# OPPO-Mente-Lab/X2I

Measured on AMD Instinct MI355X. Metric: images/sec, FLUX-schnell 1024x1024 4-step (projector + denoise loop), whole job, higher is better.
Workload: dtype bf16; 1 GPU; BASELINE configs[1]: qwen3b conditioning (C=37,H=2048,S_txt=512) -> projector -> shuttle-3/FLUX-schnell DiT 1024x1024, 4 steps; batch_per_gpu=4, global_batch=4, parallelism=batch-sharded x1, graph=True

## Files before the change

### x2i_amd/csrc/c_api.hip

```cpp
#include <stdarg.h>
#include <stdio.h>

#include "x2i_common.h"
#include "x2i_kernels.h"

static thread_local char g_err[512] = "";

int x2i_set_error(int code, const char* fmt, ...) {
  va_list ap;
  va_start(ap, fmt);
  vsnprintf(g_err, sizeof(g_err), fmt, ap);
  va_end(ap);
  return code;
}

int x2i_check_launch(const char* what) {
  hipError_t e = hipGetLastError();
  if (e != hipSuccess) return x2i_set_error(X2I_ERR_HIP, "%s: launch failed: %s", what, hipGetErrorString(e));
  return X2I_OK;
}

#include <stdlib.h>
#include <string.h>

#include <mutex>
#include <set>
#include <utility>

namespace {
int env_int(const char* name, int dflt) {
  const char* v = getenv(name);
  return v && *v ? atoi(v) : dflt;
}
X2IOptions make_options() {
  X2IOptions o;
  o.gemm_tile = env_int("X2I_GEMM_TILE", 0);
  o.gemm_min256 = env_int("X2I_GEMM_MIN256", 128);
  o.gemm_gm = env_int("X2I_GEMM_GM", 0);
  o.gemm_split_tail = env_int("X2I_GEMM_NOSPLIT", 0) ? 0 : 1;
  o.gemm_w4 = env_int("X2I_GEMM_W4", 1);
  o.gemm_persist = env_int("X2I_GEMM_PERSIST", 1);
  o.gemm_fp8_persist = env_int("X2I_GEMM_FP8_PERSIST", 1);
  o.gemm_fx = env_int("X2I_GEMM_FX", 2);
  o.gemm_fx_nk = env_int("X2I_GEMM_FX_NK", 96);
  o.gemm_streamk = env_int("X2I_GEMM_STREAMK", 1);
  o.gemm_pair = env_int("X2I_GEMM_PAIR", 1);
  o.train_rows_wg = env_int("X2I_TRAIN_ROWS_WG", 1);
  o.attn_bwd_overlap = env_int("X2I_ATTN_BWD_OVERLAP", 1);
  o.conv256 = env_int("X2I_CONV256", 1);
  o.conv_w4 = env_int("X2I_CONV_W4", 1);
  o.conv_korder = env_int("X2I_CONV_KORDER", 1);
  o.attn_variant = env_int("X2I_ATTN_VARIANT", 0);
  o.attn_w16 = env_int("X2I_ATTN_W16", 1);
  o.attn_streamk = env_int("X2I_ATTN_STREAMK", 1);
  o.conv5_variant = env_int("X2I_CONV5_VARIANT", 0);
  o.fp8 = env_int("X2I_FP8", 0);
  o.last_gemm_tile = X2I_FORM_NONE;
  o.attn_ablate = env_int("X2I_ATTN_ABLATE", 0);
  return o;
}
std::mutex g_smem_mu;
std::set<std::pair<const void*, int>> g_smem_done;
}

X2IOptions& x2i_options() {
  static X2IOptions o = make_options();
  return o;
}

int x2i_ensure_dynamic_smem(const void* kernel, int bytes) {
  int dev = 0;
  hipGetDevice(&dev);
  const std::pair<const void*, int> key(kernel, dev);
  std::lock_guard<std::mutex> lk(g_smem_mu);
  if (g_smem_done.count(key)) return X2I_OK;
  const hipError_t e = hipFuncSetAttribute(kernel, hipFuncAttributeMaxDynamicSharedMemorySize, bytes);
  if (e != hipSuccess) return x2i_set_error(X2I_ERR_HIP, "hipFuncSetAttribute(MaxDynamicSharedMemorySize=%d): %s", bytes, hipGetErrorString(e));
  g_smem_done.insert(key);
  return X2I_OK;
}

int x2i_num_cus() {
  static int cus[64] = {0};
  int dev = 0;
  hipGetDevice(&dev);
  if (dev < 0 || dev >= 64) dev = 0;
  if (!cus[dev]) {
    int n = 0;
    if (hipDeviceGetAttribute(&n, hipDeviceAttributeMultiprocessorCount, dev) != hipSuccess || n <= 0) n = 256;
    cus[dev] = n;
  }
  return cus[dev];
}

bool x2i_streamk_workspace(const x2i_gemm_args* a, float** slabs, unsigned** flags, int* rc) {
  *rc = X2I_OK;
  if (!a->workspace) return false;
  const long long need = 4096 + (long long)x2i_gemm_sk_slabs() * x2i_gemm_sk_slab_bytes();
  if (a->workspace_bytes < need || (((uintptr_t)a->workspace) & 255)) {
    *rc = x2i_set_error(X2I_ERR_ARG, "gemm: stream-K workspace must be 256-byte aligned and >= x2i_streamk_workspace_bytes() = %lld bytes (got %lld)",
                        need, (long long)a->workspace_bytes);
    return false;
  }
  *flags = (unsigned*)a->workspace;
  *slabs = (float*)((char*)a->workspace + 4096);
  return true;
}

extern "C" {

int x2i_abi_version(void) { return X2I_ABI_VERSION; }

static long long* opt_slot(X2IOptions& o, const char* name, int** as_int) {
  *as_int = nullptr;
#define X2I_OPT_INT(N_) if (!strcmp(name, #N_)) { *as_int = &o.N_; return nullptr; }
  X2I_OPT_INT(gemm_tile) X2I_OPT_INT(gemm_gm) X2I_OPT_INT(gemm_split_tail) X2I_OPT_INT(gemm_w4) X2I_OPT_INT(gemm_persist) X2I_OPT_INT(gemm_fp8_persist) X2I_OPT_INT(gemm_fx) X2I_OPT_INT(gemm_fx_nk) X2I_OPT_INT(gemm_streamk) X2I_OPT_INT(gemm_pair) X2I_OPT_INT(train_rows_wg) X2I_OPT_INT(attn_bwd_overlap) X2I_OPT_INT(attn_streamk) X2I_OPT_INT(conv256) X2I_OPT_INT(conv_w4) X2I_OPT_INT(conv_korder) X2I_OPT_INT(attn_variant) X2I_OPT_INT(attn_w16) X2I_OPT_INT(conv5_variant) X2I_OPT_INT(fp8) X2I_OPT_INT(last_gemm_tile)
#ifdef X2I_ABLATION
  X2I_OPT_INT(attn_ablate)
#endif
#undef X2I_OPT_INT
  if (!strcmp(name, "gemm_min256")) return &o.gemm_min256;
  return nullptr;
}

int x2i_set_option(const char* name, int64_t value) {
  if (!name) return x2i_set_error(X2I_ERR_ARG, "set_option: null name");
  int* ip;
  long long* lp = opt_slot(x2i_options(), name, &ip);
  if (ip) *ip = (int)value;
  else if (lp) *lp = (long long)value;
  else return x2i_set_error(X2I_ERR_ARG, "set_option: unknown option '%s'", name);
  return X2I_OK;
}

int x2i_get_option(const char* name, int64_t* value) {
  if (!name || !value) return x2i_set_error(X2I_ERR_ARG, "get_option: null pointer");
  int* ip;
  long long* lp = opt_slot(x2i_options(), name, &ip);
  if (ip) *value = *ip;
  else if (lp) *value = *lp;
  else return x2i_set_error(X2I_ERR_ARG, "get_option: unknown option '%s'", name);
  return X2I_OK;
}

int64_t x2i_streamk_workspace_bytes(void) { return 4096 + (int64_t)x2i_gemm_sk_slabs() * x2i_gemm_sk_slab_bytes(); }

int x2i_streamk_workspace_status(const void* workspace, int64_t workspace_bytes) {
  if (!workspace || workspace_bytes < x2i_streamk_workspace_bytes()) return x2i_set_error(X2I_ERR_ARG, "streamk_workspace_status: no / too small workspace");
  unsigned v = 0;
  const hipError_t e = hipMemcpy(&v, (const unsigned*)workspace + x2i_gemm_sk_max_tiles(), 4, hipMemcpyDeviceToHost);
  if (e != hipSuccess) return x2i_set_error(X2I_ERR_HIP, "streamk_workspace_status: %s", hipGetErrorString(e));
  return v ? 1 : 0;
}

int x2i_is_ablation_build(void) {
#ifdef X2I_ABLATION
  return 1;
#else
  return 0;
#endif
}
const char* x2i_last_error(void) { return g_err; }

int x2i_gemm_bf16(const x2i_gemm_args* args, x2i_stream_t stream) { return x2i_launch_gemm(args, (hipStream_t)stream); }

int x2i_gemm_fp8(const x2i_gemm_args* args, const x2i_fp8_desc* fp8, x2i_stream_t stream) {
  return x2i_launch_gemm_fp8(args, fp8, (hipStream_t)stream);
}

// ... 340 lines not shown
```

### x2i_amd/csrc/elementwise.hip

```cpp
#include "x2i_common.h"
#include "x2i_kernels.h"

namespace {

__device__ __forceinline__ void unpack8(const bf16x8_t& v, float (&f)[8]) {
#pragma unroll
  for (int i = 0; i < 8; ++i) f[i] = bf16_to_f32((bf16_t)v[i]);
}
__device__ __forceinline__ bf16x8_t pack8(const float (&f)[8]) {
  union { bf16x8_t v; uint32_t u[4]; } r;
#pragma unroll
  for (int i = 0; i < 4; ++i) r.u[i] = pack_bf16x2(f[2 * i], f[2 * i + 1]);
  return r.v;
}

constexpr int LN_MAXV = 8;

template <bool AFFINE>
__global__ __launch_bounds__(256) void ln_kernel(const bf16_t* __restrict__ X, long long x_bs, int ldx, bf16_t* __restrict__ Y,
                                                 long long y_bs, int ldy, int S, int D, int S0, const float* shift0,
                                                 const float* scale0, const float* shift1, const float* scale1,
                                                 long long mod_bs, const bf16_t* aw, const bf16_t* ab, float eps,
                                                 long long total_rows) {
  const int lane = threadIdx.x & 63;
// ... 223 lines not shown
#pragma unroll
      for (int b = 0; b < NB; ++b) acc[r][b] = 0.f;
#pragma unroll
      for (int q = 0; q < NP; ++q) acc2[r][q] = f32x2{0.f, 0.f};
    }
    for (int k = lane * 8; k < K; k += 512) {
      bf16x8_t wv[R];
#pragma unroll
      for (int r = 0; r < R; ++r) {
        const int n = min(n0 + r, N - 1);
        wv[r] = __builtin_nontemporal_load((const bf16x8_t*)(W + (long long)n * K + k));
      }
      float wf[R][8];
#pragma unroll
      for (int r = 0; r < R; ++r) unpack8(wv[r], wf[r]);
#pragma unroll
      for (int j = 0; j < 8; ++j) {
        const float* xk = xs + (k + j) * NBP;
#pragma unroll
        for (int q = 0; q < NP; ++q) {
          const f32x2 x2 = *(const f32x2*)(xk + 2 * q);
#pragma unroll
          for (int r = 0; r < R; ++r) acc2[r][q] = __builtin_elementwise_fma(f32x2{wf[r][j], wf[r][j]}, x2, acc2[r][q]);
        }
        if constexpr (NB & 1) {
          const float x1 = xk[NB - 1];
#pragma unroll
          for (int r = 0; r < R; ++r) acc[r][NB - 1] = fmaf(wf[r][j], x1, acc[r][NB - 1]);
        }
      }
    }
#pragma unroll
    for (int r = 0; r < R; ++r)
#pragma unroll
      for (int q = 0; q < NP; ++q) { acc[r][2 * q] = acc2[r][q][0]; acc[r][2 * q + 1] = acc2[r][q][1]; }
#pragma unroll
    for (int r = 0; r < R; ++r) {
#pragma unroll
      for (int b = 0; b < NB; ++b) acc[r][b] = wave_sum(acc[r][b]);
      const int n = n0 + r;
      if (lane == 0 && n < N && rr + r < rpw) {
        const float bv = bias ? bf16_to_f32(bias[n]) : 0.f;
#pragma unroll
        for (int b = 0; b < NB; ++b) {
          float v = apply_act(acc[r][b] + bv, act_out);
          float* yp = Y + (long long)b * ldy + n;
          *yp = accumulate ? (*yp + v) : v;
        }
      }
    }
  }
}

__global__ void sinusoid_kernel(const float* __restrict__ t, float* __restrict__ out, int B, int dim, int round_bf16) {
  const int i = blockIdx.x * blockDim.x + threadIdx.x;
  const int half = dim / 2;
  if (i >= B * dim) return;
  const int b = i / dim, j = i - b * dim;
  const int k = j < half ? j : j - half;
  const float f = expf(-logf(10000.f) * (float)k / (float)half);
  const float a = t[b] * f;
  float v = j < half ? cosf(a) : sinf(a);
  if (round_bf16) v = bf16_to_f32(f32_to_bf16(v));
  out[i] = v;
}

__global__ void rope_table_kernel(const float* __restrict__ ids, int S, int d0, int d1, int d2, double theta, float* __restrict__ cosp,
                                  float* __restrict__ sinp) {
  const int D = d0 + d1 + d2;
  const long long i = (long long)blockIdx.x * blockDim.x + threadIdx.x;
  if (i >= (long long)S * D) return;
  const int s = (int)(i / D), c = (int)(i - (long long)s * D);
  int a = 0, start = 0, d = d0;
  if (c >= d0 + d1) a = 2, start = d0 + d1, d = d2;
  else if (c >= d0) a = 1, start = d0, d = d1;
  const int k = (c - start) >> 1;
  const double freq = 1.0 / pow(theta, (double)(2 * k) / (double)d);
  const double ang = (double)ids[(long long)s * 3 + a] * freq;
  cosp[i] = (float)cos(ang);
  sinp[i] = (float)sin(ang);
}

__global__ void euler_kernel(bf16_t* __restrict__ x, const bf16_t* __restrict__ eps, long long n8, const float* __restrict__ dt) {
  const float d = dt[0];
  for (long long i = (long long)blockIdx.x * blockDim.x + threadIdx.x; i < n8; i += (long long)gridDim.x * blockDim.x) {
    float a[8], e[8];
    unpack8(*(const bf16x8_t*)(x + i * 8), a);
    unpack8(*(const bf16x8_t*)(eps + i * 8), e);
#pragma unroll
    for (int j = 0; j < 8; ++j) a[j] = a[j] + d * e[j];
    *(bf16x8_t*)(x + i * 8) = pack8(a);
  }
}

__global__ __launch_bounds__(256) void gated_residual_kernel(bf16_t* __restrict__ X, long long x_bs, int ldx, const bf16_t* __restrict__ T,
                                                             long long t_bs, int ldt, const float* __restrict__ gate, long long g_bs, int S,
                                                             int D8, long long total) {
  for (long long i = (long long)blockIdx.x * blockDim.x + threadIdx.x; i < total; i += (long long)gridDim.x * blockDim.x) {
    const int c = (int)(i % D8);
    const long long row = i / D8;
    const int b = (int)(row / S), s = (int)(row - (long long)b * S);
    bf16_t* x = X + (long long)b * x_bs + (long long)s * ldx + c * 8;
    float a[8], t[8];
    unpack8(*(const bf16x8_t*)x, a);
    unpack8(*(const bf16x8_t*)(T + (long long)b * t_bs + (long long)s * ldt + c * 8), t);
    const float* g = gate + (long long)b * g_bs + c * 8;
// ... 38 lines not shown
  if (ldx % 8 || ldy % 8 || x_bs % 8 || y_bs % 8 || mod_bs % 4 || !al16(X) || !al16(Y)) return x2i_set_error(X2I_ERR_ALIGN, "ln_modulate: rows must be 16-byte aligned");
  const long long rows = (long long)B * S;
  if (D == 3072 && rows >= 4096) {
    hipLaunchKernelGGL((ln_rows_kernel<6, 4>), dim3((unsigned)((rows + 15) / 16)), dim3(256), 0, stream, (const bf16_t*)X, x_bs, ldx, (bf16_t*)Y, y_bs,
                       ldy, S, S0, shift0 ? shift0 : shift1, scale0 ? scale0 : scale1, shift1, scale1, mod_bs, eps, rows);
    return x2i_check_launch("ln_modulate");
  }
  hipLaunchKernelGGL(ln_kernel<false>, dim3((unsigned)((rows + 3) / 4)), dim3(256), 0, stream, (const bf16_t*)X, x_bs, ldx,
                     (bf16_t*)Y, y_bs, ldy, S, D, S0, shift0 ? shift0 : shift1, scale0 ? scale0 : scale1, shift1, scale1, mod_bs,
                     (const bf16_t*)nullptr, (const bf16_t*)nullptr, eps, rows);
  return x2i_check_launch("ln_modulate");
}

int x2i_launch_ln_affine(const void* X, void* Y, long long rows, int D, const void* w, const void* b, float eps, hipStream_t stream) {
  if (!X || !Y || !w || !b) return x2i_set_error(X2I_ERR_ARG, "ln_affine: null pointer");
  if (D % 8 || D > 64 * 8 * LN_MAXV || rows <= 0) return x2i_set_error(X2I_ERR_SHAPE, "ln_affine: D=%d unsupported", D);
  if (!al16(X) || !al16(Y) || !al16(w) || !al16(b)) return x2i_set_error(X2I_ERR_ALIGN, "ln_affine: 16-byte alignment required");
  hipLaunchKernelGGL(ln_kernel<true>, dim3((unsigned)((rows + 3) / 4)), dim3(256), 0, stream, (const bf16_t*)X, (long long)0, D,
                     (bf16_t*)Y, (long long)0, D, (int)1 << 30, D, 0, (const float*)nullptr, (const float*)nullptr,
                     (const float*)nullptr, (const float*)nullptr, (long long)0, (const bf16_t*)w, (const bf16_t*)b, eps, rows);
  return x2i_check_launch("ln_affine");
}

int x2i_launch_qkv_split(const void* qkv0, const void* qkv1, int ld0, int ld1, int B, int S, int S0, int H, const void* nq0,
                         const void* nk0, const void* nq1, const void* nk1, const float* cosp, const float* sinp, void* Q,
                         void* K, void* VT, int Spad, float eps, hipStream_t stream) {
  if (S0 < 0 || S0 > S || B <= 0 || S <= 0 || H <= 0) return x2i_set_error(X2I_ERR_SHAPE, "qkv_split: bad shape");
  if ((S0 > 0 && (!qkv0 || !nq0 || !nk0)) || (S0 < S && (!qkv1 || !nq1 || !nk1)) || !cosp || !sinp || !Q || !K || !VT)
    return x2i_set_error(X2I_ERR_ARG, "qkv_split: null pointer");
  if (Spad % 128 || Spad < S) return x2i_set_error(X2I_ERR_SHAPE, "qkv_split: Spad=%d must be a multiple of 128 and >= S=%d", Spad, S);
  if ((S0 > 0 && ld0 % 8) || (S0 < S && ld1 % 8)) return x2i_set_error(X2I_ERR_ALIGN, "qkv_split: ld must be a multiple of 8");
  hipLaunchKernelGGL(qk_norm_rope_kernel, dim3(S, B), dim3(256), 0, stream, (const bf16_t*)qkv0, (const bf16_t*)qkv1, ld0, ld1, S,
                     S0, H, (const bf16_t*)nq0, (const bf16_t*)nk0, (const bf16_t*)nq1, (const bf16_t*)nk1, cosp, sinp, (bf16_t*)Q,
                     (bf16_t*)K, Spad, eps);
  int rc = x2i_check_launch("qk_norm_rope");
  if (rc) return rc;
  hipLaunchKernelGGL(v_transpose_kernel, dim3((S + 63) / 64, H, B), dim3(256), 0, stream, (const bf16_t*)qkv0, (const bf16_t*)qkv1,
                     ld0, ld1, S, S0, H, (bf16_t*)VT, Spad);
  return x2i_check_launch("v_transpose");
}

int x2i_launch_skinny_linear(const void* X, int x_is_bf16, const void* W, const void* bias, float* Y, int ldy, int B, int N, int K,
                             int act_in, int act_out, int accumulate, hipStream_t stream) {
  return x2i_launch_skinny_linear_grouped(X, x_is_bf16, 0, W, bias, Y, ldy, 1, B, N, K, act_in, act_out, accumulate, stream);
}

int x2i_launch_skinny_linear_grouped(const void* X, int x_is_bf16, long long x_gs, const void* W, const void* bias, float* Y, int ldy, int G, int B,
                                     int N, int K, int act_in, int act_out, int accumulate, hipStream_t stream) {
  if (!X || !W || !Y) return x2i_set_error(X2I_ERR_ARG, "skinny_linear: null pointer");
  if (G <= 0 || G > 65535 || x_gs < 0) return x2i_set_error(X2I_ERR_SHAPE, "skinny_linear: bad group count / stride (G=%d)", G);
  if (G > 1 && B > SK_MAXB) return x2i_set_error(X2I_ERR_SHAPE, "skinny_linear_grouped: at most %d rows per group (B=%d)", SK_MAXB, B);
  if (B <= 0 || N <= 0 || K <= 0 || K % 8) return x2i_set_error(X2I_ERR_SHAPE, "skinny_linear: K=%d must be a multiple of 8", K);
  if (!al16(W)) return x2i_set_error(X2I_ERR_ALIGN, "skinny_linear: W must be 16-byte aligned");
  const int esz = x_is_bf16 ? 2 : 4;
  for (int b0 = 0; b0 < B; b0 += SK_MAXB) {
    const int nb = (B - b0) < SK_MAXB ? (B - b0) : SK_MAXB;
    const void* xp = (const char*)X + (long long)b0 * K * esz;
    float* yp = Y + (long long)b0 * ldy;
    const int rpw = N >= 65536 ? 16 : 4;
    const dim3 grid((N + 4 * rpw - 1) / (4 * rpw), G), block(256);
    const size_t shm = (size_t)(nb == 1 ? 1 : (nb + 1) & ~1) * K * 4;
    if (shm > 160 * 1024) return x2i_set_error(X2I_ERR_SHAPE, "skinny_linear: B*K too large for LDS");
#define SK_CASE(NB)                                                                                                   \
  case NB: {                                                                                                          \
    hipError_t e = hipFuncSetAttribute((const void*)skinny_linear_kernel<NB>, hipFuncAttributeMaxDynamicSharedMemorySize, \
                                       (int)shm);                                                                     \
    if (e != hipSuccess) return x2i_set_error(X2I_ERR_HIP, "skinny_linear: %s", hipGetErrorString(e));                \
    hipLaunchKernelGGL(skinny_linear_kernel<NB>, grid, block, shm, stream, xp, x_is_bf16, (const bf16_t*)W,           \
                       (const bf16_t*)bias, yp, ldy, N, K, act_in, act_out, accumulate, rpw, x_gs, B);               \
  } break;
    switch (nb) {
      SK_CASE(1) SK_CASE(2) SK_CASE(3) SK_CASE(4) SK_CASE(5) SK_CASE(6) SK_CASE(7) SK_CASE(8)
    }
#undef SK_CASE
    int rc = x2i_check_launch("skinny_linear");
    if (rc) return rc;
  }
  return X2I_OK;
}

int x2i_launch_timestep_sinusoid(const float* t, float* out, int B, int dim, int round_bf16, hipStream_t stream) {
  if (!t || !out || B <= 0 || dim <= 0 || dim % 2) return x2i_set_error(X2I_ERR_ARG, "timestep_sinusoid: bad argument");
  hipLaunchKernelGGL(sinusoid_kernel, dim3((B * dim + 255) / 256), dim3(256), 0, stream, t, out, B, dim, round_bf16);
  return x2i_check_launch("timestep_sinusoid");
}

int x2i_launch_rope_table(const float* ids, int S, int d0, int d1, int d2, float theta, float* cosp, float* sinp, hipStream_t stream) {
  if (!ids || !cosp || !sinp || S <= 0) return x2i_set_error(X2I_ERR_ARG, "rope_table: bad argument");
  if (d0 < 0 || d1 < 0 || d2 < 0 || (d0 | d1 | d2) & 1 || d0 + d1 + d2 <= 0 || theta <= 0.f)
    return x2i_set_error(X2I_ERR_SHAPE, "rope_table: axis dims must be even and non-negative (%d,%d,%d)", d0, d1, d2);
  const long long n = (long long)S * (d0 + d1 + d2);
  hipLaunchKernelGGL(rope_table_kernel, dim3((unsigned)((n + 255) / 256)), dim3(256), 0, stream, ids, S, d0, d1, d2, (double)theta, cosp, sinp);
  return x2i_check_launch("rope_table");
}

int x2i_launch_gated_residual(void* X, long long x_bs, int ldx, const void* T, long long t_bs, int ldt, const float* gate, long long g_bs,
                              int B, int S, int D, hipStream_t stream) {
  if (!X || !T || !gate || B <= 0 || S <= 0 || D <= 0) return x2i_set_error(X2I_ERR_ARG, "gated_residual: bad argument");
  if (D % 8 || ldx % 8 || ldt % 8 || x_bs % 8 || t_bs % 8 || g_bs % 4 || !al16(X) || !al16(T) || !al16(gate))
    return x2i_set_error(X2I_ERR_ALIGN, "gated_residual: rows must be 16-byte aligned, D %% 8 == 0");
  const long long total = (long long)B * S * (D / 8);
  const long long blocks = (total + 255) / 256;
  hipLaunchKernelGGL(gated_residual_kernel, dim3((unsigned)(blocks < 8192 ? blocks : 8192)), dim3(256), 0, stream, (bf16_t*)X, x_bs, ldx,
                     (const bf16_t*)T, t_bs, ldt, gate, g_bs, S, D / 8, total);
  return x2i_check_launch("gated_residual");
}
// ... 36 lines not shown
```

### x2i_amd/csrc/x2i_common.h

```cpp
#pragma once
#include <hip/hip_runtime.h>
#include <stdint.h>

typedef uint16_t bf16_t;
typedef __attribute__((ext_vector_type(8))) short bf16x8_t;
typedef __attribute__((ext_vector_type(4))) short bf16x4_t;
typedef __attribute__((ext_vector_type(4))) float f32x4_t;
typedef __attribute__((ext_vector_type(16))) float f32x16_t;

#define X2I_OK 0
#define X2I_ERR_ARG (-1)
#define X2I_ERR_SHAPE (-2)
#define X2I_ERR_ALIGN (-3)
#define X2I_ERR_HIP (-4)
#define X2I_ERR_STATE (-5)

int x2i_set_error(int code, const char* fmt, ...);
int x2i_check_launch(const char* what);

struct X2IOptions {
  int gemm_tile;
  long long gemm_min256;
  int gemm_gm;
  int gemm_split_tail;
  int gemm_w4;
  int attn_bwd_overlap;
  int train_rows_wg;
  int gemm_pair;
  int gemm_streamk;
  int gemm_fx_nk;
  int gemm_fx;
  int gemm_fp8_persist;
  int gemm_persist;
  int conv256;
  int conv_w4;
  int conv_korder;
  int attn_variant;
  int attn_w16;
  int attn_streamk;
  int conv5_variant;
  int fp8;
  int last_gemm_tile;
  int attn_ablate;
};
X2IOptions& x2i_options();
enum X2IGemmForm {
  X2I_FORM_NONE = -1,
  X2I_FORM_GENERIC = 0,
  X2I_FORM_128 = 128,
  X2I_FORM_256 = 256,
  X2I_FORM_256_TAIL = 1256,
  X2I_FORM_PAIR = 2256,
  X2I_FORM_FX = 3256,
  X2I_FORM_CONV256C = 5256,
  X2I_FORM_CONV512C = 5512,
  X2I_FORM_FP8 = 7256,
  X2I_FORM_FP8_PERSIST = 8256,
  X2I_FORM_FP8_STREAMK = 9256,
};
int x2i_ensure_dynamic_smem(const void* kernel, int bytes);
int x2i_num_cus();
struct x2i_gemm_args;
bool x2i_streamk_workspace(const x2i_gemm_args* a, float** slabs, unsigned** flags, int* rc);
long long x2i_conv_moments_scratch(int M, int N, int batch);
int x2i_conv_moments_reduce(float* scratch, float* moments, int batch, int blocks, int N, int accumulate, hipStream_t stream);
int x2i_gemm_sk_slabs();
int x2i_gemm_sk_max_tiles();
long long x2i_gemm_sk_slab_bytes();

__device__ __forceinline__ int x2i_vt_pos(int t, int perm) {
  return perm ? ((t & ~31) | (((t >> 2) & 3) << 3) | (((t >> 4) & 1) << 2) | (t & 3)) : t;
}
__device__ __forceinline__ float bf16_to_f32(bf16_t v) { return __uint_as_float(((uint32_t)v) << 16); }
__device__ __forceinline__ bf16_t f32_to_bf16(float f) {
  const __bf16 h = (__bf16)f;
  return __builtin_bit_cast(unsigned short, h);
}
__device__ __forceinline__ uint32_t pack_bf16x2(float lo, float hi) {
  typedef __attribute__((ext_vector_type(2))) __bf16 bf16x2_hw;
  typedef __attribute__((ext_vector_type(2))) float f32x2_hw;
  const f32x2_hw v = {lo, hi};
  const bf16x2_hw h = __builtin_convertvector(v, bf16x2_hw);
  return __builtin_bit_cast(uint32_t, h);
}
__device__ __forceinline__ float xhalf_max(float x) {
  const auto r = __builtin_amdgcn_permlane32_swap(__float_as_uint(x), __float_as_uint(x), false, false);
  return fmaxf(__uint_as_float(r[0]), __uint_as_float(r[1]));
}
__device__ __forceinline__ float xhalf_sum(float x) {
  const auto r = __builtin_amdgcn_permlane32_swap(__float_as_uint(x), __float_as_uint(x), false, false);
  return __uint_as_float(r[0]) + __uint_as_float(r[1]);
}
__device__ __forceinline__ float gelu_tanh_f(float x) {
  const float z = x * __builtin_fmaf(x * x, -0.10294324f, -2.3022082f);
// ... 73 lines not shown
```

### x2i_amd/flux.py

```python
import math
import os
from typing import Optional

import torch
import torch.nn as nn

from . import ops
from .ops import ACT_GELU_TANH, ACT_NONE, ACT_SILU


class _P(nn.Module):

    def __init__(self, **tensors):
        super().__init__()
        for k, v in tensors.items():
            self.register_parameter(k, nn.Parameter(v, requires_grad=False))


class _AttnTap(nn.Module):

    def forward(self, *outs):
        return outs if len(outs) > 1 else outs[0]


# ... 213 lines not shown
            S=S, Spad=Spad,
            X=torch.empty((B, S, D), **bf), NRM=torch.empty((B, S, D), **bf), QKV=torch.empty((B * S, 3 * D), **bf),
            Q=torch.zeros((B, H, Spad, 128), **bf), K=torch.zeros((B, H, Spad, 128), **bf),
            VT=torch.zeros((B, H, 128, Spad), **bf), ATT=torch.empty((B, S, D), **bf),
            CAT=torch.empty((B * S, 5 * D), **bf), NRMF=torch.empty((B * Si, D), **bf),
            MOD=torch.empty((B, self._mod_rows), device=dev, dtype=torch.float32),
            TEMB=torch.empty((B, D), device=dev, dtype=torch.float32),
            H1=torch.empty((B, D), device=dev, dtype=torch.float32),
        )
        if self._fp8 is not None:
            f8 = dict(device=dev, dtype=ops.FP8)
            ws.update(NRM8=torch.empty((B, S, D), **f8), RS=torch.empty((B * S,), device=dev, dtype=torch.float32),
                      H8=torch.empty((B * Si, 4 * D), **f8), CAT8=torch.empty((B * S, 5 * D), **f8))
            if self._fp8_mode == "all":
                ws.update(ATT8=torch.empty((B, S, D), **f8))
        self._ws = {key: ws}
        return ws

    @torch.no_grad()
    def prepare_conditioning(self, encoder_hidden_states, pooled_projections, txt_ids, img_ids, guidance=None):
        cfg = self.config
        D = self.inner_dim
        enc = encoder_hidden_states
        B, St, Kj = enc.shape
        if txt_ids.ndim == 3:
            txt_ids = txt_ids[0]
        if img_ids.ndim == 3:
            img_ids = img_ids[0]
        Si = img_ids.shape[0]
        ws = self._workspace(B, St, Si)
        S = ws["S"]
        f = self._fused
        enc = enc.to(device=self.device, dtype=torch.bfloat16).contiguous()
        ctx = torch.empty((B, St, D), device=self.device, dtype=torch.bfloat16)
        ops.gemm(enc, f["context_embedder.w"], f["context_embedder.b"], out=ctx, M=B * St)
        ids = torch.cat((txt_ids.to(self.device), img_ids.to(self.device)), dim=0)
        cos, sin = ops.rope_table(ids, cfg.axes_dims_rope)
        pairs = ops.rope_pairs(cos, sin, check=False)
        cond = torch.empty((B, D), device=self.device, dtype=torch.float32)
        pooled = pooled_projections.to(device=self.device, dtype=torch.bfloat16).contiguous()
        h1 = ops.skinny_linear(pooled, f["tte.text_embedder.1.w"], f["tte.text_embedder.1.b"], out=ws["H1"], act_out=ACT_SILU)
        ops.skinny_linear(h1, f["tte.text_embedder.2.w"], f["tte.text_embedder.2.b"], out=cond)
        if cfg.guidance_embeds:
            if guidance is None:
                raise ValueError("guidance is required when config.guidance_embeds is True")
            g = (guidance.to(device=self.device, dtype=pooled_projections.dtype) * 1000).float().contiguous()
            gp = ops.timestep_sinusoid(g, 256, round_bf16=pooled_projections.dtype == torch.bfloat16)
            h1 = ops.skinny_linear(gp, f["tte.guidance_embedder.1.w"], f["tte.guidance_embedder.1.b"], out=ws["H1"], act_out=ACT_SILU)
            ops.skinny_linear(h1, f["tte.guidance_embedder.2.w"], f["tte.guidance_embedder.2.b"], out=cond, accumulate=True)
        return dict(B=B, St=St, Si=Si, ctx=ctx, cos=cos, sin=sin, rope_pairs=pairs, cond=cond, ws=ws,
                    round_bf16=pooled_projections.dtype == torch.bfloat16)

    MOD_GROUP = 4

    @torch.no_grad()
    def prepare_modulation(self, state, timesteps, dtype=torch.bfloat16):
        f = self._fused
        B, n = state["B"], len(timesteps)
        g = self.MOD_GROUP // B
        if g < 2:
            return [None] * n
        out = []
        for i0 in range(0, n, g):
            ts = timesteps[i0:i0 + g]
            t1000 = torch.cat([(t.to(device=self.device, dtype=dtype) * 1000).float().reshape(-1).expand(B) for t in ts]).contiguous()
            tp = ops.timestep_sinusoid(t1000, 256, round_bf16=state["round_bf16"])
            h1 = ops.skinny_linear(tp, f["tte.timestep_embedder.1.w"], f["tte.timestep_embedder.1.b"], act_out=ACT_SILU)
            temb = state["cond"].repeat(len(ts), 1)
            ops.skinny_linear(h1, f["tte.timestep_embedder.2.w"], f["tte.timestep_embedder.2.b"], out=temb, accumulate=True)
            table = ops.skinny_linear(temb, f["mod.w"], f["mod.b"], act_in=ACT_SILU)
            out += [table[k * B:(k + 1) * B] for k in range(len(ts))]
        return out

    @torch.no_grad()
    def denoise(self, state, hidden_states, timestep, control=None, mod=None):
        cfg = self.config
        f = self._fused
        ws = state["ws"]
        B, St, Si = state["B"], state["St"], state["Si"]
        S, Spad = ws["S"], ws["Spad"]
        D, H = self.inner_dim, self._H
        X, NRM, QKV, Q, K, VT, ATT, CAT, MOD = (ws[k] for k in ("X", "NRM", "QKV", "Q", "K", "VT", "ATT", "CAT", "MOD"))
        Ntot = self._mod_rows
        hs = hidden_states.to(device=self.device, dtype=torch.bfloat16).contiguous()
        X[:, :St].copy_(state["ctx"])
        ops.gemm(hs, f["x_embedder.w"], f["x_embedder.b"], out=X, M=Si, batch=B, a_batch_stride=Si * cfg.in_channels,
                 lda=cfg.in_channels, c_batch_stride=S * D, ldc=D, c_offset=St * D)
        t1000 = None
        if mod is None or control is not None:
            t1000 = (timestep.to(device=self.device, dtype=hidden_states.dtype) * 1000).float().contiguous()
        if mod is not None:
            MOD = mod
        else:
            tp = ops.timestep_sinusoid(t1000, 256, round_bf16=state["round_bf16"])
            h1 = ops.skinny_linear(tp, f["tte.timestep_embedder.1.w"], f["tte.timestep_embedder.1.b"], out=ws["H1"], act_out=ACT_SILU)
            temb = ws["TEMB"]
            temb.copy_(state["cond"])
            ops.skinny_linear(h1, f["tte.timestep_embedder.2.w"], f["tte.timestep_embedder.2.b"], out=temb, accumulate=True)
            ops.skinny_linear(temb, f["mod.w"], f["mod.b"], out=MOD, act_in=ACT_SILU)
        cos, sin = state["cos"], state["sin"]
        rc, rs = (state["rope_pairs"], None) if self.rope_pair_tables else (cos, sin)
        scale = 1.0 / math.sqrt(128.0)

        def mod(off):
            return MOD[:, off:]

        fuse_qkv = self.fuse_qkv and D % 64 == 0
        fp8 = self._fp8
        fp8_all = fp8 is not None and self._fp8_mode == "all"
        qs = scale * 1.4426950408889634 if (fuse_qkv or fp8_all) else 1.0
        scale = scale / qs if qs != 1.0 else scale
        vp_d = fuse_qkv and not fp8_all and ops.attention_prefers_vt_perm(H, S, scale)
        vp_s = fuse_qkv and fp8 is None and ops.attention_prefers_vt_perm(H, S, scale)
        taps = any(len(b.attn._forward_hooks) for b in self.transformer_blocks) or \
            any(len(b.attn._forward_hooks) for b in self.single_transformer_blocks)
        if taps and fp8 is not None:
            raise RuntimeError("attention taps (forward hooks on block.attn) are served by the bf16 configuration only")
# ... 211 lines not shown
```

### x2i_amd/pipeline.py

```python
import math
from typing import Optional

import os

import numpy as np
import torch

from . import ops


class FlowMatchEulerDiscreteScheduler:

    def __init__(self, num_train_timesteps: int = 1000, shift: float = 1.0, use_dynamic_shifting: bool = False,
                 base_shift: float = 0.5, max_shift: float = 1.15, base_image_seq_len: int = 256,
                 max_image_seq_len: int = 4096):
        self.config = _Cfg(num_train_timesteps=num_train_timesteps, shift=shift, use_dynamic_shifting=use_dynamic_shifting,
                           base_shift=base_shift, max_shift=max_shift, base_image_seq_len=base_image_seq_len,
                           max_image_seq_len=max_image_seq_len)
        ts = np.linspace(1, num_train_timesteps, num_train_timesteps, dtype=np.float32)[::-1].copy()
        sig = ts / num_train_timesteps
        if not use_dynamic_shifting:
            sig = shift * sig / (1 + (shift - 1) * sig)
        self.sigma_min, self.sigma_max = float(sig[-1]), float(sig[0])
        self.timesteps = torch.from_numpy(sig * num_train_timesteps)
# ... 139 lines not shown

    @torch.no_grad()
    def __call__(self, prompt_embeds=None, pooled_prompt_embeds=None, num_inference_steps: int = 28,
                 guidance_scale: float = 3.5, height: Optional[int] = None, width: Optional[int] = None,
                 output_type: str = "latent", generator=None, latents=None, guided_hint=None, use_graph: bool = False,
                 return_dict: bool = True, **unused):
        if prompt_embeds is None or pooled_prompt_embeds is None:
            raise ValueError("x2i_amd FluxPipeline is driven by prompt_embeds/pooled_prompt_embeds (no text encoders), "
                             "as every reference inference script does")
        if output_type != "latent":
            raise ValueError('only output_type="latent" is on the hot path (VAE decode is the caller\'s, as in the reference)')
        tr = self.transformer
        ops.streamk_check(sync=False)
        height = height or self.default_sample_size * self.vae_scale_factor
        width = width or self.default_sample_size * self.vae_scale_factor
        if height % 16 or width % 16:
            raise ValueError("height and width must be multiples of 16")
        device = tr.device
        dtype = prompt_embeds.dtype
        B = prompt_embeds.shape[0]
        prompt_embeds = prompt_embeds.to(device)
        pooled_prompt_embeds = pooled_prompt_embeds.to(device)
        txt_ids = torch.zeros(prompt_embeds.shape[1], 3, device=device, dtype=dtype)
        C = tr.config.in_channels // 4
        latents, img_ids = self.prepare_latents(B, C, height, width, dtype, device, generator, latents)
        sc = self.scheduler.config
        sigmas = np.linspace(1.0, 1 / num_inference_steps, num_inference_steps)
        mu = calculate_shift(latents.shape[1], sc.base_image_seq_len, sc.max_image_seq_len, sc.base_shift, sc.max_shift)
        self.scheduler.set_timesteps(sigmas=sigmas, device=device, mu=mu)
        timesteps = self.scheduler.timesteps
        guidance = None
        if tr.config.guidance_embeds:
            guidance = torch.full([1], guidance_scale, device=device, dtype=torch.float32).expand(B)
        hint = guided_hint.to(device) if (self.control_nets is not None and guided_hint is not None) else None
        latents = latents.contiguous()
        if latents.dtype != torch.bfloat16:
            state = tr.prepare_conditioning(prompt_embeds, pooled_prompt_embeds, txt_ids, img_ids, guidance)
            control = self._control_fn(hint)
            for i, t in enumerate(timesteps):
                ts = t.expand(B).to(latents.dtype)
                noise = tr.denoise(state, latents, ts / 1000, control=control)
                latents = self.scheduler.step(noise.to(latents.dtype), t, latents)[0]
            return FluxPipelineOutput(latents) if return_dict else (latents,)

        dts = (self.scheduler.sigmas[1:] - self.scheduler.sigmas[:-1]).to(device=device, dtype=torch.float32).contiguous()
        tvals = [(t.expand(B).to(torch.bfloat16) / 1000).contiguous() for t in timesteps]

        aux = dict(txt_ids=txt_ids, img_ids=img_ids, guidance=guidance, dts=dts, tvals=tvals,
                   ws=tr._workspace(B, prompt_embeds.shape[1], latents.shape[1]))

        def body(pe, pooled, lat, hnt):
            state = tr.prepare_conditioning(pe, pooled, aux["txt_ids"], aux["img_ids"], aux["guidance"])
            control = self._control_fn(hnt)
            mods = tr.prepare_modulation(state, tvals, lat.dtype) if self.hoist_modulation else [None] * len(tvals)
            for i in range(len(tvals)):
                noise = tr.denoise(state, lat, tvals[i], control=control, mod=mods[i])
                ops.euler_step_(lat, noise, dts[i:i + 1])

        key = (B, prompt_embeds.shape[1], height, width, num_inference_steps, float(guidance_scale), hint is not None,
               getattr(self.transformer, "_fp8_mode", None),
               self.hoist_modulation,
               ops.option_epoch())
        entry = self._graphs.get(key) if use_graph else None
        if entry is None and not (use_graph and key in self._seen):
            latents = latents.clone()
            body(prompt_embeds, pooled_prompt_embeds, latents, hint)
            ops.streamk_poll()
            self.graph_stats["eager"] += 1
            self._seen[key] = True
            while len(self._seen) > 256:
                self._seen.pop(next(iter(self._seen)))
            return FluxPipelineOutput(latents) if return_dict else (latents,)
        if entry is None:
            torch.cuda.synchronize(device)
            torch.cuda.empty_cache()
            before = torch.cuda.memory_reserved(device)
            static = dict(pe=prompt_embeds.clone(), pooled=pooled_prompt_embeds.clone(), lat=latents.clone(),
                          hint=None if hint is None else hint.clone())
            aux["sk_ws"] = ops.StreamKWorkspace(device)
            graph = torch.cuda.CUDAGraph()
            with torch.cuda.graph(graph), ops.streamk_scope(aux["sk_ws"]):
                body(static["pe"], static["pooled"], static["lat"], static["hint"])
            torch.cuda.synchronize(device)
            nbytes = max(0, torch.cuda.memory_reserved(device) - before)
            entry = [graph, static, aux, nbytes]
            self._graphs[key] = entry
            self.graph_stats["captures"] += 1
            self._evict(keep=key)
        else:
            self._graphs[key] = self._graphs.pop(key)
        graph, static = entry[0], entry[1]
        static["pe"].copy_(prompt_embeds)
        static["pooled"].copy_(pooled_prompt_embeds)
        static["lat"].copy_(latents)
        if hint is not None:
            static["hint"].copy_(hint)
        graph.replay()
        entry[2]["sk_ws"].poll()
        self.graph_stats["replays"] += 1
        out = static["lat"].clone()
        return FluxPipelineOutput(out) if return_dict else (out,)

    def _evict(self, keep=None):
        def total():
            return sum(e[3] for e in self._graphs.values())
        while len(self._graphs) > 1 and (len(self._graphs) > self.graph_cache_entries or total() > self.graph_cache_bytes):
            victim = next(k for k in self._graphs if k != keep)
# ... 38 lines not shown
```

Baseline: 4.576 images/s.

## Batch modulation across timesteps with a wide multi-row skinny linear kernel

Adds a persistent skinny-linear kernel that handles up to 16 rows per launch, streaming weight tiles through a double-buffered LDS ring and reducing with permlane and DPP ops. Modulation hoisting now groups up to 16 rows, so with batch 4 all four timesteps' modulation is computed in one pass instead of per step. This reads the large modulation weights once rather than per timestep, at the cost of a new kernel path and more working memory.

```diff
diff --git a/x2i_amd/csrc/c_api.hip b/x2i_amd/csrc/c_api.hip
--- a/x2i_amd/csrc/c_api.hip
+++ b/x2i_amd/csrc/c_api.hip
@@ -54,8 +54,10 @@
   o.attn_w16 = env_int("X2I_ATTN_W16", 1);
   o.attn_streamk = env_int("X2I_ATTN_STREAMK", 1);
   o.conv5_variant = env_int("X2I_CONV5_VARIANT", 0);
+  o.skinny_wide = env_int("X2I_SKINNY_WIDE", 1);
   o.fp8 = env_int("X2I_FP8", 0);
   o.last_gemm_tile = X2I_FORM_NONE;
+  o.last_skinny_wide = 0;
   o.attn_ablate = env_int("X2I_ATTN_ABLATE", 0);
   return o;
 }
@@ -114,7 +116,7 @@
 static long long* opt_slot(X2IOptions& o, const char* name, int** as_int) {
   *as_int = nullptr;
 #define X2I_OPT_INT(N_) if (!strcmp(name, #N_)) { *as_int = &o.N_; return nullptr; }
-  X2I_OPT_INT(gemm_tile) X2I_OPT_INT(gemm_gm) X2I_OPT_INT(gemm_split_tail) X2I_OPT_INT(gemm_w4) X2I_OPT_INT(gemm_persist) X2I_OPT_INT(gemm_fp8_persist) X2I_OPT_INT(gemm_fx) X2I_OPT_INT(gemm_fx_nk) X2I_OPT_INT(gemm_streamk) X2I_OPT_INT(gemm_pair) X2I_OPT_INT(train_rows_wg) X2I_OPT_INT(attn_bwd_overlap) X2I_OPT_INT(attn_streamk) X2I_OPT_INT(conv256) X2I_OPT_INT(conv_w4) X2I_OPT_INT(conv_korder) X2I_OPT_INT(attn_variant) X2I_OPT_INT(attn_w16) X2I_OPT_INT(conv5_variant) X2I_OPT_INT(fp8) X2I_OPT_INT(last_gemm_tile)
+  X2I_OPT_INT(gemm_tile) X2I_OPT_INT(gemm_gm) X2I_OPT_INT(gemm_split_tail) X2I_OPT_INT(gemm_w4) X2I_OPT_INT(gemm_persist) X2I_OPT_INT(gemm_fp8_persist) X2I_OPT_INT(gemm_fx) X2I_OPT_INT(gemm_fx_nk) X2I_OPT_INT(gemm_streamk) X2I_OPT_INT(gemm_pair) X2I_OPT_INT(train_rows_wg) X2I_OPT_INT(attn_bwd_overlap) X2I_OPT_INT(attn_streamk) X2I_OPT_INT(conv256) X2I_OPT_INT(conv_w4) X2I_OPT_INT(conv_korder) X2I_OPT_INT(attn_variant) X2I_OPT_INT(attn_w16) X2I_OPT_INT(conv5_variant) X2I_OPT_INT(skinny_wide) X2I_OPT_INT(fp8) X2I_OPT_INT(last_gemm_tile) X2I_OPT_INT(last_skinny_wide)
 #ifdef X2I_ABLATION
   X2I_OPT_INT(attn_ablate)
 #endif
diff --git a/x2i_amd/csrc/elementwise.hip b/x2i_amd/csrc/elementwise.hip
--- a/x2i_amd/csrc/elementwise.hip
+++ b/x2i_amd/csrc/elementwise.hip
@@ -299,6 +299,159 @@
   }
 }
 
+constexpr int SKW_MAXB = 16;
+constexpr int SKW_MAXK = 3072;
+constexpr int SKW_THREADS = SKW_MAXB / 2 * 64;
+constexpr int SKW_R = 4;
+constexpr int SKW_NW = SKW_MAXK / 512;
+constexpr int SKW_TILE = SKW_R * SKW_MAXK / 8;
+constexpr int SKW_Q = SKW_TILE / SKW_THREADS;
+constexpr int SKW_MAXIT = 2048;
+constexpr int SKW_MIN_N = 65536;
+
+__device__ __forceinline__ float skw_fold32(float a, float b) {
+  const auto r = __builtin_amdgcn_permlane32_swap(__float_as_uint(a), __float_as_uint(b), false, false);
+  return __uint_as_float(r[0]) + __uint_as_float(r[1]);
+}
+__device__ __forceinline__ float skw_fold16(float a, float b) {
+  const auto r = __builtin_amdgcn_permlane16_swap(__float_as_uint(a), __float_as_uint(b), false, false);
+  return __uint_as_float(r[0]) + __uint_as_float(r[1]);
+}
+template <int CTRL>
+__device__ __forceinline__ float skw_dpp(float v) {
+  return __builtin_bit_cast(float, __builtin_amdgcn_update_dpp(0, __builtin_bit_cast(int, v), CTRL, 0xf, 0xf, true));
+}
+__device__ __forceinline__ float skw_tail8(float a, float b, int lane) {
+  const bool hi = lane & 8;
+  float z = (hi ? b : a) + skw_dpp<0x128>(hi ? a : b);
+  const float up = skw_dpp<0x104>(z), dn = skw_dpp<0x114>(z);
+  z = z + (lane & 4 ? dn : up);
+  z = z + skw_dpp<0x4E>(z);
+  z = z + skw_dpp<0xB1>(z);
+  return z;
+}
+
+template <bool FULLK>
+__global__ __launch_bounds__(SKW_THREADS) void skinny_linear_wide_kernel(const void* __restrict__ Xv, int x_is_bf16,
+                                                                         const bf16_t* __restrict__ W, const bf16_t* __restrict__ bias,
+                                                                         float* __restrict__ Y, int ldy, int B, int N, int K, int act_in,
+                                                                         int act_out, int accumulate) {
+  typedef float f32x2 __attribute__((ext_vector_type(2)));
+  __shared__ __attribute__((aligned(16))) bf16x8_t ring[2][SKW_TILE];
+  __shared__ bf16_t lbias[SKW_MAXIT * SKW_R];
+  const bf16x8_t zeros = {0, 0, 0, 0, 0, 0, 0, 0};
+  const int tid = threadIdx.x, lane = tid & 63, wave = tid >> 6;
+  const int b0 = wave * 2;
+  const bool active = b0 < B;
+  const bool silu = act_in == X2I_ACT_SILU;
+  f32x2 xp[SKW_NW][8];
+#pragma unroll
+  for (int i = 0; i < SKW_NW; ++i) {
+    const int k0 = lane * 8 + i * 512;
+#pragma unroll
+    for (int h = 0; h < 2; ++h) {
+      const long long idx = (long long)(b0 + h < B ? b0 + h : B - 1) * K + (k0 < K ? k0 : 0);
+#pragma unroll
+      for (int j = 0; j < 8; ++j) xp[i][j][h] = x_is_bf16 ? bf16_to_f32(((const bf16_t*)Xv)[idx + j]) : ((const float*)Xv)[idx + j];
+    }
+  }
+#pragma unroll
+  for (int i = 0; i < SKW_NW; ++i)
+#pragma unroll
+    for (int h = 0; h < 2; ++h) {
+      const bool live = b0 + h < B && lane * 8 + i * 512 < K;
+#pragma unroll
+      for (int j = 0; j < 8; ++j) xp[i][j][h] = live ? (silu ? silu_f(xp[i][j][h]) : xp[i][j][h]) : 0.f;
+    }
+  const int cpt = K >> 1;
+  const long long wchunks = ((long long)N * K) >> 3;
+  const int ntiles = (N + SKW_R - 1) / SKW_R;
+  const int nit = (ntiles - (int)blockIdx.x + (int)gridDim.x - 1) / (int)gridDim.x;
+  const bf16x8_t* W8 = (const bf16x8_t*)W;
+  if (bias)
+    for (int e = tid; e < nit * SKW_R; e += SKW_THREADS) {
+      const long long n = ((long long)blockIdx.x + (long long)(e / SKW_R) * gridDim.x) * SKW_R + e % SKW_R;
+      lbias[e] = n < N ? bias[n] : (bf16_t)0;
+    }
+  auto fetch = [&](bf16x8_t (&s)[SKW_Q], int it) {
+    const long long base = ((long long)blockIdx.x + (long long)it * gridDim.x) * cpt;
+#pragma unroll
+    for (int q = 0; q < SKW_Q; ++q) {
+      const int c = tid + SKW_THREADS * q;
+      const bool live = c < cpt && base + c < wchunks;
+      s[q] = __builtin_nontemporal_load(W8 + (live ? base + c : wchunks - 1));
+    }
+  };
+  auto stash = [&](int slot, const bf16x8_t (&s)[SKW_Q]) {
+#pragma unroll
+    for (int q = 0; q < SKW_Q; ++q) ring[slot][tid + SKW_THREADS * q] = s[q];
+  };
+  auto barrier = [&]() { asm volatile("s_waitcnt lgkmcnt(0)\n\ts_barrier" ::: "memory"); };
+  const int er = ((lane >> 5) & 1) * 2 + ((lane >> 4) & 1), eb = b0 + ((lane >> 3) & 1);
+  const bool writer = active && !(lane & 7) && eb < B;
+
+  auto emit = [&](int it, float z) {
+    const int n = ((int)blockIdx.x + it * (int)gridDim.x) * SKW_R + er;
+    if (writer && n < N) {
+      const float bv = bias ? bf16_to_f32(lbias[it * SKW_R + er]) : 0.f;
+      float v = apply_act(z + bv, act_out);
+      float* yp = Y + (long long)eb * ldy + n;
+      *yp = accumulate ? (*yp + v) : v;
+    }
+  };
+
+  auto iter = [&](int it, bf16x8_t (&s1)[SKW_Q]) {
+    stash((it + 1) & 1, s1);
+    fetch(s1, it + 3);
+    if (active) {
+      const bf16x8_t* tile = ring[it & 1];
+      f32x2 acc[SKW_R];
+#pragma unroll
+      for (int r = 0; r < SKW_R; ++r) acc[r] = f32x2{0.f, 0.f};
+#pragma unroll
+      for (int i = 0; i < SKW_NW; ++i) {
+        bf16x8_t wv[SKW_R];
+#pragma unroll
+        for (int r = 0; r < SKW_R; ++r) wv[r] = FULLK || lane * 8 + i * 512 < K ? tile[((r * K) >> 3) + lane + i * 64] : zeros;
+#pragma unroll
+        for (int j = 0; j < 8; ++j) {
+#pragma unroll
+          for (int r = 0; r < SKW_R; ++r) {
+            const float w = bf16_to_f32((bf16_t)wv[r][j]);
+            acc[r][0] = fmaf(w, xp[i][j][0], acc[r][0]);
+            acc[r][1] = fmaf(w, xp[i][j][1], acc[r][1]);
+          }
+          __builtin_amdgcn_sched_barrier(0);
+        }
+      }
+      float u[4], t[2];
+#pragma unroll
+      for (int v = 0; v < 4; ++v) u[v] = skw_fold32(acc[v >> 1][v & 1], acc[2 + (v >> 1)][v & 1]);
+#pragma unroll
+      for (int v = 0; v < 2; ++v) t[v] = skw_fold16(u[v], u[v + 2]);
+      emit(it, skw_tail8(t[0], t[1], lane));
+    }
+    barrier();
+  };
+
+  bf16x8_t sa[SKW_Q], sb[SKW_Q];
+  fetch(sa, 0);
+  fetch(sb, 1);
+  stash(0, sa);
+  fetch(sa, 2);
+  barrier();
+#pragma unroll 1
+  for (int it = 0; it < nit; it += 4) {
+    iter(it, sb);
+    if (it + 1 >= nit) break;
+    iter(it + 1, sa);
+    if (it + 2 >= nit) break;
+    iter(it + 2, sb);
+    if (it + 3 >= nit) break;
+    iter(it + 3, sa);
+  }
+}
+
 __global__ void sinusoid_kernel(const float* __restrict__ t, float* __restrict__ out, int B, int dim, int round_bf16) {
   const int i = blockIdx.x * blockDim.x + threadIdx.x;
   const int half = dim / 2;
@@ -443,6 +596,20 @@
   if (G > 1 && B > SK_MAXB) return x2i_set_error(X2I_ERR_SHAPE, "skinny_linear_grouped: at most %d rows per group (B=%d)", SK_MAXB, B);
   if (B <= 0 || N <= 0 || K <= 0 || K % 8) return x2i_set_error(X2I_ERR_SHAPE, "skinny_linear: K=%d must be a multiple of 8", K);
   if (!al16(W)) return x2i_set_error(X2I_ERR_ALIGN, "skinny_linear: W must be 16-byte aligned");
+  const int wide = x2i_options().skinny_wide;
+  if (G == 1 && B > 4 && B <= SKW_MAXB && K <= SKW_MAXK && (act_in == X2I_ACT_NONE || act_in == X2I_ACT_SILU) && wide > 0 &&
+      (wide >= 2 || N >= SKW_MIN_N) && (N + SKW_R - 1) / SKW_R <= (long long)SKW_MAXIT * x2i_num_cus()) {
+    const int ntiles = (N + SKW_R - 1) / SKW_R, cus = x2i_num_cus();
+    x2i_options().last_skinny_wide = 1;
+    if (K == SKW_MAXK)
+      hipLaunchKernelGGL(skinny_linear_wide_kernel<true>, dim3(ntiles < cus ? ntiles : cus), dim3(SKW_THREADS), 0, stream, X, x_is_bf16, (const bf16_t*)W,
+                         (const bf16_t*)bias, Y, ldy, B, N, K, act_in, act_out, accumulate);
+    else
+    hipLaunchKernelGGL(skinny_linear_wide_kernel<false>, dim3(ntiles < cus ? ntiles : cus), dim3(SKW_THREADS), 0, stream, X, x_is_bf16, (const bf16_t*)W,
+                       (const bf16_t*)bias, Y, ldy, B, N, K, act_in, act_out, accumulate);
+    return x2i_check_launch("skinny_linear_wide");
+  }
+  x2i_options().last_skinny_wide = 0;
   const int esz = x_is_bf16 ? 2 : 4;
   for (int b0 = 0; b0 < B; b0 += SK_MAXB) {
     const int nb = (B - b0) < SK_MAXB ? (B - b0) : SK_MAXB;
diff --git a/x2i_amd/csrc/x2i_common.h b/x2i_amd/csrc/x2i_common.h
--- a/x2i_amd/csrc/x2i_common.h
+++ b/x2i_amd/csrc/x2i_common.h
@@ -39,7 +39,9 @@
   int attn_w16;
   int attn_streamk;
   int conv5_variant;
+  int skinny_wide;
   int fp8;
+  int last_skinny_wide;
   int last_gemm_tile;
   int attn_ablate;
 };
diff --git a/x2i_amd/flux.py b/x2i_amd/flux.py
--- a/x2i_amd/flux.py
+++ b/x2i_amd/flux.py
@@ -289,17 +289,25 @@
                     round_bf16=pooled_projections.dtype == torch.bfloat16)
 
     MOD_GROUP = 4
+    MOD_ROWS = 16
+
+    @classmethod
+    def modulation_passes(cls, B, n, rows=None):
+        if rows is None or B == 1 or not ops._lib.get_option("skinny_wide"):
+            rows = cls.MOD_GROUP
+        g = max(1, min(rows, cls.MOD_ROWS) // B)
+        return g, [(i0, min(g, n - i0)) for i0 in range(0, n, g)]
 
     @torch.no_grad()
-    def prepare_modulation(self, state, timesteps, dtype=torch.bfloat16):
+    def prepare_modulation(self, state, timesteps, dtype=torch.bfloat16, rows=None):
         f = self._fused
         B, n = state["B"], len(timesteps)
-        g = self.MOD_GROUP // B
+        g, passes = self.modulation_passes(B, n, rows)
         if g < 2:
             return [None] * n
         out = []
-        for i0 in range(0, n, g):
-            ts = timesteps[i0:i0 + g]
+        for i0, cnt in passes:
+            ts = timesteps[i0:i0 + cnt]
             t1000 = torch.cat([(t.to(device=self.device, dtype=dtype) * 1000).float().reshape(-1).expand(B) for t in ts]).contiguous()
             tp = ops.timestep_sinusoid(t1000, 256, round_bf16=state["round_bf16"])
             h1 = ops.skinny_linear(tp, f["tte.timestep_embedder.1.w"], f["tte.timestep_embedder.1.b"], act_out=ACT_SILU)
diff --git a/x2i_amd/pipeline.py b/x2i_amd/pipeline.py
--- a/x2i_amd/pipeline.py
+++ b/x2i_amd/pipeline.py
@@ -215,7 +215,7 @@
         def body(pe, pooled, lat, hnt):
             state = tr.prepare_conditioning(pe, pooled, aux["txt_ids"], aux["img_ids"], aux["guidance"])
             control = self._control_fn(hnt)
-            mods = tr.prepare_modulation(state, tvals, lat.dtype) if self.hoist_modulation else [None] * len(tvals)
+            mods = tr.prepare_modulation(state, tvals, lat.dtype, rows=tr.MOD_ROWS) if self.hoist_modulation else [None] * len(tvals)
             for i in range(len(tvals)):
                 noise = tr.denoise(state, lat, tvals[i], control=control, mod=mods[i])
                 ops.euler_step_(lat, noise, dts[i:i + 1])
```

Result: no change. 4.598 images/s, median of 6 (+0.5%).
